# songrise/AvatarCraft

Measured on AMD Instinct MI355X. Metric: rays/sec, 4096-ray batch, 256x256 render (64+64 samples/ray), higher is better.
Workload: dtype f32

## Files before the change

avatarcraft_amd/csrc/nsr_device.hpp:

```cpp
#pragma once
#include "ac_common.hpp"
#include "ac_devmath.hpp"
#include "ac_sp_table.hpp"
#include "ac_sh16.hpp"
#include <type_traits>

using namespace acdev;

typedef float f32x4 __attribute__((ext_vector_type(4)));

namespace {

#ifndef AC_WPB
#define AC_WPB 8
#endif
constexpr int WAVES_PER_BLOCK = AC_WPB;
constexpr int BLOCK = WAVES_PER_BLOCK * 64;
#ifndef AC_MAXT
#define AC_MAXT 128
#endif
constexpr int MAXT = AC_MAXT;
constexpr int SEG_STATE = MAXT + 16 + 64;
#ifndef AC_ENC_ROUND
#define AC_ENC_ROUND 2
#endif

constexpr int OFF_W1F = 0;
constexpr int OFF_W2F = OFF_W1F + 4 * 9 * 64;
constexpr int OFF_C1F = OFF_W2F + 16 * 64;
constexpr int OFF_C2F = OFF_C1F + 4 * 6 * 64;
constexpr int OFF_C3F = OFF_C2F + 4 * 16 * 64;
constexpr int OFF_B1 = OFF_C3F + 16 * 64;
constexpr int OFF_B2 = OFF_B1 + 64;
constexpr int OFF_LVL = OFF_B2 + 16;
constexpr int OFF_LIN = OFF_LVL + 16 * 8;
constexpr int SPQ_FLOATS = 129 * 4;
constexpr int OFF_SPQ = OFF_LIN + 80;
constexpr int OFF_WAVE = OFF_SPQ + SPQ_FLOATS;
constexpr int FE_SLAB = 6 * 8 * 64;
constexpr int OFF_W1H = OFF_WAVE;
constexpr int OFF_W1L = OFF_W1H + 4 * 64 * 4;
constexpr int OFF_W1C = OFF_W1L + 4 * 64 * 4;
constexpr int CF_FRAGS = 14, CF_FRAG = 64 * 4;
constexpr int OFF_CFH = OFF_C1F;
constexpr int OFF_CFL = OFF_C1F + CF_FRAGS * CF_FRAG;
constexpr int OFF_C3L = OFF_W1C + 3 * 64;
static_assert(OFF_CFL + 12 * CF_FRAG == OFF_B1, "the bf16 colour fragments fill the fp32 colour region exactly");
constexpr int OFF_RWAVE = OFF_C3L + 2 * CF_FRAG;
constexpr int CF_OVERLAY = OFF_B1 - OFF_C1F;
constexpr int UPS_FLOATS = MAXT + 2 * MAXT + MAXT + 32;
constexpr int SLAB_ACC = MAXT + (FE_SLAB > UPS_FLOATS ? FE_SLAB : UPS_FLOATS);
constexpr int SLAB_SHB = SLAB_ACC + 16;
constexpr int WAVE_SLAB = SLAB_SHB + 80;
constexpr int LDS_FLOATS = OFF_RWAVE + WAVES_PER_BLOCK * WAVE_SLAB;
static_assert(LDS_FLOATS * 4 <= 160 * 1024, "LDS budget: one workgroup per CU");
static_assert(OFF_WAVE % 4 == 0 && OFF_RWAVE % 4 == 0 && WAVE_SLAB % 4 == 0, "16-byte aligned slabs");

#ifdef AC_PROFILE
#define AC_T0() unsigned long long t_prof_ = __builtin_amdgcn_s_memtime(); const unsigned long long ray_r0_ = __builtin_amdgcn_s_memrealtime()
#define AC_TICK(SLOT) { const unsigned long long t2_ = __builtin_amdgcn_s_memtime(); prof_acc[SLOT] += t2_ - t_prof_; t_prof_ = t2_; }
#else
#define AC_T0()
#define AC_TICK(SLOT)
#endif

struct LevelRec { float scale; uint32_t my, mz, offset, mask, hashed, wsize, pad; };

struct RenderArgs {
    const float *table;
    uint32_t table_bytes;
    const float *W1, *b1, *W2, *b2, *Wc1, *Wc2, *Wc3;
    const float *Wsh;
    const float *prepared;
    const float *rays_o, *rays_d, *bg, *noise, *lin_z, *lin_u;
    ac_render_out out;
    LevelRec lvl[16];
    int n_rays, T0, nup;
    int jmode[4];
    int jfine[4];
    float bound, two_bound, inv_s, car, one_m_car, eps;
    float inv_tb;
    const float *inv_s_dev;
    int fast;
    int skip_masked;
    int opacity_only;
    int perturb;
    unsigned long long *prof;
    const float *near_m, *far_m;
    const float *ext_pts;
    const uint8_t *mask;
    uint32_t *ray_counter;
    uint32_t *seg_flags;
    float *seg_state;
    uint64_t seg_cb;
    int seg_n;
    int pair_n;
    uint32_t *done_counter;
    uint32_t *handoff_timeouts;
    float *eik_red;
    uint32_t gen;
    int ex_from;
    int ex_rows;
    const uint8_t *ray_dead;
    float *zbuf;
    float *mid_pts;
};

enum { MODE_FULL = 0, MODE_UPSAMPLE = 2, MODE_FINAL = 3 };

__device__ __forceinline__ void cube_near_far(float ox, float oy, float oz, float dx, float dy, float dz, float bound, float &near, float &far)
{
    const float ex = dx + 1e-15f, ey = dy + 1e-15f, ez = dz + 1e-15f;
    const float ax = (-bound - ox) / ex, bx = (bound - ox) / ex;
    const float ay = (-bound - oy) / ey, by = (bound - oy) / ey;
    const float az = (-bound - oz) / ez, bz = (bound - oz) / ez;
    const float lx = ax < bx ? ax : bx, hx = ax > bx ? ax : bx;
    const float ly = ay < by ? ay : by, hy = ay > by ? ay : by;
    const float lz = az < bz ? az : bz, hz = az > bz ? az : bz;
    near = lx; if (ly > near) near = ly; if (lz > near) near = lz;
    far = hx; if (hy < far) far = hy; if (hz < far) far = hz;
    if (near < 0.05f) near = 0.05f;
}
__device__ __forceinline__ bool is_inf(float v) { return __builtin_fabsf(v) == __builtin_inff(); }

__device__ __forceinline__ void wave_sync()
{
    __builtin_amdgcn_fence(__ATOMIC_ACQ_REL, "wavefront");
    __builtin_amdgcn_wave_barrier();
}

template <int OFF> __device__ __forceinline__ float dpp_shr(float ident, float v)
{
    return __builtin_bit_cast(float, __builtin_amdgcn_update_dpp(__builtin_bit_cast(int, ident), __builtin_bit_cast(int, v),
                                                                  0x110 + OFF, 0xf, 0xf, false));
}
template <bool MUL> __device__ __forceinline__ float row_scan(float v)
{
    const float id = MUL ? 1.0f : 0.0f;
    float s;
    s = dpp_shr<1>(id, v); v = MUL ? s * v : s + v;
    s = dpp_shr<2>(id, v); v = MUL ? s * v : s + v;
    s = dpp_shr<4>(id, v); v = MUL ? s * v : s + v;
    s = dpp_shr<8>(id, v); v = MUL ? s * v : s + v;
    return v;
}
__device__ __forceinline__ float lane_bcast(float v, int lane)
{
    return __builtin_bit_cast(float, __builtin_amdgcn_readlane(__builtin_bit_cast(int, v), lane));
// ... 758 lines not shown
```

avatarcraft_amd/csrc/render_fused.hip:

```cpp
#include <atomic>
#include <map>
#include <mutex>
#include "nsr_device.hpp"

namespace {

#ifndef AC_XCD_CHUNK
#define AC_XCD_CHUNK 512
#endif
#define AC_RENDER_KERNEL render_rays_kernel
#define AC_RENDER_H16 false
#include "render_rays_kernel.hpp"
#undef AC_RENDER_KERNEL
#undef AC_RENDER_H16
#define AC_RENDER_KERNEL render_rays_h16_kernel
#define AC_RENDER_H16 true
#include "render_rays_kernel.hpp"
#undef AC_RENDER_KERNEL
#undef AC_RENDER_H16

__global__ __launch_bounds__(BLOCK) void field_sdf_kernel(const RenderArgs a, const float *__restrict__ x, uint32_t B,
                                                          float *__restrict__ out16)
{
    extern __shared__ __attribute__((aligned(16))) float lds[];
    fill_lds(lds, a);
    __syncthreads();
    const int lane = threadIdx.x & 63, wave = threadIdx.x >> 6, n = lane & 15, g = lane >> 4;
    const FieldCtx fc = make_ctx(a);
    const uint32_t ntiles = (B + 15) / 16;
    for (uint32_t tile = blockIdx.x * WAVES_PER_BLOCK + wave; tile < ntiles; tile += gridDim.x * WAVES_PER_BLOCK) {
        const uint32_t b = tile * 16 + n, bb = b < B ? b : B - 1;
        const float px = x[3 * bb], py = x[3 * bb + 1], pz = x[3 * bb + 2];
        const f32x4 o = sdf_tile(lds, fc, lane, px, py, pz);
        if (b < B) *reinterpret_cast<f32x4 *>(out16 + (size_t)b * 16 + 4 * g) = o;
    }
}

__global__ __launch_bounds__(BLOCK) void field_color_kernel(const RenderArgs a, const float *__restrict__ x, const float *__restrict__ dirs,
                                                            const float *__restrict__ nrm, const float *__restrict__ sdfout,
                                                            uint32_t B, float *__restrict__ rgb_out)
{
    extern __shared__ __attribute__((aligned(16))) float lds[];
    fill_lds(lds, a);
    __syncthreads();
    const int lane = threadIdx.x & 63, wave = threadIdx.x >> 6, n = lane & 15, g = lane >> 4;
    const uint32_t ntiles = (B + 15) / 16;
    float *slab = lds + OFF_WAVE + wave * 1024;
    for (uint32_t tile = blockIdx.x * WAVES_PER_BLOCK + wave; tile < ntiles; tile += gridDim.x * WAVES_PER_BLOCK) {
        const uint32_t b = tile * 16 + n, bb = b < B ? b : B - 1;
        const f32x4 so = *reinterpret_cast<const f32x4 *>(sdfout + (size_t)bb * 16 + 4 * g);
        float rgb[3];
        if (dirs) {
            wave_sync();
            sample_sh_bias(slab, a.Wsh, dirs[3 * bb], dirs[3 * bb + 1], dirs[3 * bb + 2], lane);
            color_tile(lds, lane, x[3 * bb], x[3 * bb + 1], x[3 * bb + 2], nrm[3 * bb], nrm[3 * bb + 1], nrm[3 * bb + 2], so, rgb, slab + 4 * lane, 256);
        } else
        color_tile(lds, lane, x[3 * bb], x[3 * bb + 1], x[3 * bb + 2], nrm[3 * bb], nrm[3 * bb + 1], nrm[3 * bb + 2], so, rgb);
        if (b < B && g == 0) { rgb_out[3 * b] = rgb[0]; rgb_out[3 * b + 1] = rgb[1]; rgb_out[3 * b + 2] = rgb[2]; }
    }
}

__global__ __launch_bounds__(BLOCK) void field_prepare_kernel(const RenderArgs a, float *__restrict__ image)
// ... 42 lines not shown
    const int ray = idx / T0, i = idx - ray * T0;
    const float ox = rays_o[3 * ray], oy = rays_o[3 * ray + 1], oz = rays_o[3 * ray + 2];
    const float dx = rays_d[3 * ray], dy = rays_d[3 * ray + 1], dz = rays_d[3 * ray + 2];
    float near, far;
    cube_near_far(ox, oy, oz, dx, dy, dz, bound, near, far);
    if (near_m) {
        const float nm = near_m[ray], fm = far_m[ray];
        if (!is_inf(nm)) near = nm;
        if (!is_inf(fm)) far = fm;
    }
    const float span = far - near;
    const float sample_dist = span / (float)T0;
    float zi = near + span * lin_z[i];
    if (perturb) zi = zi + (noise[idx] - 0.5f) * sample_dist;
    pts[3 * (size_t)idx] = ox + dx * zi; pts[3 * (size_t)idx + 1] = oy + dy * zi; pts[3 * (size_t)idx + 2] = oz + dz * zi;
}

static int check_render_args(const char *who, const ac_render_opts *op, const float *rays_o, const float *rays_d, const float *noise,
                             const float *lin_z, const float *lin_u, const ac_render_out *out)
{
    if (op->num_steps % 16 || op->upsample_steps % 16 || op->num_steps < 16 || op->num_steps > 64 ||
        op->upsample_steps < 0 || op->num_steps + op->upsample_steps > MAXT) {
        ac::set_error("%s: num_steps=%d upsample_steps=%d unsupported (multiples of 16, num_steps<=64, sum<=128)", who,
                      op->num_steps, op->upsample_steps);
        return AC_ERR_BAD_ARG;
    }
    if (!(op->fd_eps > 0.0f)) {
        ac::set_error("%s: fd_eps = %g (normal_epsilon_ratio >= 1): the finite-difference normals divide by it, it must be positive", who, (double)op->fd_eps);
        return AC_ERR_BAD_ARG;
    }
    if (op->n_rays <= 0) return AC_OK;
    if (!rays_o || !rays_d || !lin_z || (op->upsample_steps && !lin_u) || (op->perturb && !noise) || !out->image ||
        !out->weights_sum || !out->depth || !out->normal_map || !out->eik) {
        ac::set_error("%s: NULL buffer", who); return AC_ERR_BAD_ARG;
    }
    return AC_OK;
}

static int fill_render_args(RenderArgs &a, const ac_field *field, const ac_render_opts *op, const float *rays_o, const float *rays_d,
                            const float *bg, const float *noise, const float *lin_z, const float *lin_u, const ac_render_out *out)
{
    if (int rc = fill_render_common(a, field, op, rays_o, rays_d, bg, noise, lin_z, lin_u)) return rc;
    a.out = *out;
    a.pair_n = 0; a.ex_from = 0; a.ex_rows = op->n_rays;
    if (op->precision != 0 && op->precision != 1) { ac::set_error("ac_render_opts: precision %d unknown (0 = exact, 1 = fast)", op->precision); return AC_ERR_BAD_ARG; }
    if (op->skip_masked != 0 && op->skip_masked != 1) { ac::set_error("ac_render_opts: skip_masked must be 0 or 1"); return AC_ERR_BAD_ARG; }
    a.skip_masked = op->skip_masked;
    if (op->opacity_only != 0 && op->opacity_only != 1) { ac::set_error("ac_render_opts: opacity_only must be 0 or 1"); return AC_ERR_BAD_ARG; }
    a.opacity_only = op->opacity_only;
    if ((op->near_m != nullptr) != (op->far_m != nullptr)) { ac::set_error("ac_render_opts: near_m and far_m go together"); return AC_ERR_BAD_ARG; }
    return AC_OK;
}

#ifndef AC_RAY_SEGMENTS
#define AC_RAY_SEGMENTS 4
#endif
struct SegSlot { char *p; size_t bytes; uint32_t gen; uint64_t last_use; };
constexpr size_t SEG_POOL_MAX = 32;
static std::mutex g_seg_mu;
static std::map<std::pair<int, hipStream_t>, SegSlot> g_seg_pool;
static uint64_t g_seg_clock = 0;
static char *seg_scratch(size_t need, uint32_t &gen, hipStream_t stream)
{
    std::mutex &mu = g_seg_mu;
    auto &pool = g_seg_pool;
    int dev = 0;
    if (hipGetDevice(&dev) != hipSuccess || dev < 0) dev = 0;
    std::lock_guard<std::mutex> lock(mu);
    const auto key = std::make_pair(dev, stream);
    if (pool.find(key) == pool.end() && pool.size() >= SEG_POOL_MAX) {
        auto victim = pool.begin();
        for (auto it = pool.begin(); it != pool.end(); ++it) if (it->second.last_use < victim->second.last_use) victim = it;
        if (victim->second.p) (void)hipFree(victim->second.p);
        pool.erase(victim);
    }
    SegSlot &sl = pool[key];
    sl.last_use = ++g_seg_clock;
    if (sl.bytes < need) {
        if (sl.p) (void)hipFree(sl.p);
        sl.p = nullptr; sl.bytes = 0; sl.gen = 0;
        const size_t want = (need + ((size_t)1 << 20) - 1) & ~(((size_t)1 << 20) - 1);
        if (hipMalloc(reinterpret_cast<void **>(&sl.p), want) != hipSuccess) { sl.p = nullptr; return nullptr; }
        if (hipMemsetAsync(sl.p, 0, want, stream) != hipSuccess) { (void)hipFree(sl.p); sl.p = nullptr; return nullptr; }
        sl.bytes = want;
    }
    sl.gen = (sl.gen + 1u) & 0x0fffffffu;
    if (sl.gen == 0u) {
        if (hipMemsetAsync(sl.p, 0, sl.bytes, stream) != hipSuccess) return nullptr;
        sl.gen = 1u;
    }
    gen = sl.gen;
    return sl.p;
}

AC_API int ac_render_handoff_timeouts(ac_stream_t stream, uint32_t *count)
{
    if (!count) { ac::set_error("render_handoff_timeouts: NULL count"); return AC_ERR_BAD_ARG; }
    *count = 0;
    int dev = 0;
    if (hipGetDevice(&dev) != hipSuccess || dev < 0) dev = 0;
    char *p = nullptr;
    {
        std::lock_guard<std::mutex> lock(g_seg_mu);
        auto it = g_seg_pool.find(std::make_pair(dev, (hipStream_t)stream));
        if (it != g_seg_pool.end()) p = it->second.p;
    }
    if (!p) return AC_OK;
    if (hipMemcpyAsync(count, p + 260, sizeof(uint32_t), hipMemcpyDeviceToHost, (hipStream_t)stream) != hipSuccess ||
        hipStreamSynchronize((hipStream_t)stream) != hipSuccess) { ac::set_error("render_handoff_timeouts: copy failed"); return AC_ERR_LAUNCH; }
    return AC_OK;
}

template <int MODE, bool FAST, bool EX, bool SH = false, bool H16 = false>
static void launch_render_p(const RenderArgs &a, hipStream_t stream)
{
    const auto kernel = H16 ? render_rays_h16_kernel<MODE, FAST, EX, SH> : render_rays_kernel<MODE, FAST, EX, SH>;
    int blocks = (a.n_rays + WAVES_PER_BLOCK - 1) / WAVES_PER_BLOCK;
    static uint64_t seen = 0;
    const size_t lds_bytes = LDS_FLOATS * sizeof(float);
    ac::allow_dynamic_lds(seen, reinterpret_cast<const void *>(kernel), lds_bytes);
    RenderArgs b = a;
    {
        const int nt = (a.T0 + 16 * a.nup) / 16;
        int sn = (MODE != MODE_FULL) ? 1 : (nt < AC_RAY_SEGMENTS ? nt : AC_RAY_SEGMENTS);
        if (sn < 1) sn = 1;
        b.seg_n = sn; b.seg_cb = 0;
        for (int q = 0; q <= sn; ++q) b.seg_cb |= (uint64_t)((nt * q) / sn) << (4 * q);
        const size_t N = (size_t)a.n_rays, head = 512, flags = (N * 4 + 255) & ~(size_t)255;
        const size_t need = head + (sn > 1 ? flags + N * SEG_STATE * sizeof(float) : 0);
        uint32_t gen = 0;
        char *sc = seg_scratch(need, gen, stream);
        b.ray_counter = reinterpret_cast<uint32_t *>(sc);
        b.done_counter = sc ? reinterpret_cast<uint32_t *>(sc + 256) : nullptr;
        b.handoff_timeouts = sc ? reinterpret_cast<uint32_t *>(sc + 260) : nullptr;
        b.gen = gen;
        b.eik_red = (MODE == MODE_UPSAMPLE) ? nullptr : a.out.eik_reduced;
        b.seg_flags = sn > 1 ? reinterpret_cast<uint32_t *>(sc + head) : nullptr;
        b.seg_state = sn > 1 ? reinterpret_cast<float *>(sc + head + flags) : nullptr;
        const int cus = (int)ac::cu_count();
        if (blocks > cus) blocks = cus;
        blocks = (blocks + 7) & ~7;
        if (!sc) blocks = 0;
    }
    hipLaunchKernelGGL(kernel, dim3(blocks), dim3(BLOCK), lds_bytes, stream, b);
}
static bool wants_samples(const ac_render_out &o)
{
    return o.z_vals || o.weights || o.alpha || o.color || o.sdf || o.gradient || o.ss_inds || o.sort_index || o.sdf_out16 || o.pts || o.feat7;
}
template <int MODE>
static void launch_render(const RenderArgs &a, hipStream_t stream, bool h16 = false)
{
    const bool ex = wants_samples(a.out);
    if constexpr (MODE != MODE_UPSAMPLE) {
        dispatch_variants(a.fast, ex, a.Wsh != nullptr, [&](auto fast, auto ex_, auto sh) {
            if (h16) launch_render_p<MODE, decltype(fast)::value, decltype(ex_)::value, decltype(sh)::value, true>(a, stream);
            else launch_render_p<MODE, decltype(fast)::value, decltype(ex_)::value, decltype(sh)::value>(a, stream);
        });
        return;
    }
    const bool inds = a.out.ss_inds || a.out.sort_index;
    if (h16) { if (inds) launch_render_p<MODE, false, true, false, true>(a, stream); else launch_render_p<MODE, false, false, false, true>(a, stream); }
    else if (inds) launch_render_p<MODE, false, true>(a, stream);
    else launch_render_p<MODE, false, false>(a, stream);
}

__global__ __launch_bounds__(256) void table_to_half_kernel(const float2 *__restrict__ table, uint32_t n_entries, uint32_t *__restrict__ out, uint32_t *__restrict__ n_bad)
{
    uint32_t bad = 0;
    for (uint32_t i = blockIdx.x * blockDim.x + threadIdx.x; i < n_entries; i += gridDim.x * blockDim.x) {
        const float2 v = table[i];
        const _Float16 h0 = (_Float16)v.x, h1 = (_Float16)v.y;
        const uint32_t b0 = __builtin_bit_cast(unsigned short, h0), b1 = __builtin_bit_cast(unsigned short, h1);
        out[i] = b0 | (b1 << 16);
        const bool o0 = (b0 & 0x7fffu) == 0x7c00u && !is_inf(v.x), o1 = (b1 & 0x7fffu) == 0x7c00u && !is_inf(v.y);
        bad += (o0 || o1) ? 1u : 0u;
    }
    if (bad) atomicAdd(n_bad, bad);
}

AC_API int ac_table_to_half(const float *table, uint32_t n_entries, void *table_h16, uint32_t *n_bad, ac_stream_t stream)
{
    if (n_entries == 0) return AC_OK;
    if (!table || !table_h16 || !n_bad) { ac::set_error("table_to_half: NULL buffer"); return AC_ERR_BAD_ARG; }
    uint32_t blocks = (n_entries + 255u) / 256u;
    if (blocks > 4096u) blocks = 4096u;
    hipLaunchKernelGGL(table_to_half_kernel, dim3(blocks), dim3(256), 0, (hipStream_t)stream, reinterpret_cast<const float2 *>(table), n_entries,
                       static_cast<uint32_t *>(table_h16), n_bad);
    return ac::check_launch("table_to_half");
}

static int check_h16_args(const char *who, const ac_field *field, const void *table_h16, const ac_render_opts *op, const ac_render_out *out)
{
    if (!field) { ac::set_error("%s: NULL field", who); return AC_ERR_BAD_ARG; }
// ... 282 lines not shown
```

avatarcraft_amd/csrc/render_rays_kernel.hpp:

```cpp
template <int MODE, bool FAST, bool EX, bool SH = false>
__global__ __launch_bounds__(BLOCK) void AC_RENDER_KERNEL(const RenderArgs a)
{
    constexpr bool FC = FAST;
    extern __shared__ __attribute__((aligned(16))) float lds[];
    if (a.prepared) {
        const float4 *src = reinterpret_cast<const float4 *>(a.prepared);
        float4 *dst = reinterpret_cast<float4 *>(lds);
        for (int e = threadIdx.x; e < OFF_RWAVE / 4; e += blockDim.x)
            dst[e] = src[(FC && 4 * e >= OFF_C1F && 4 * e < OFF_B1) ? e + (OFF_RWAVE - OFF_C1F) / 4 : e];
        __syncthreads();
        for (int e = threadIdx.x; e < 64; e += blockDim.x) lds[OFF_LIN + e] = e < a.T0 ? a.lin_z[e] : 0.0f;
        for (int e = threadIdx.x; e < 16; e += blockDim.x) lds[OFF_LIN + 64 + e] = a.lin_u ? a.lin_u[e] : 0.0f;
    } else {
        fill_lds_sdf(lds, a);
        if constexpr (FAST) fill_lds_fast(lds, a);
        if constexpr (FC) fill_lds_color_fast<true, true>(lds, a);
        else fill_lds_color(lds, a);
    }
    __syncthreads();

    const int lane = threadIdx.x & 63, wave = threadIdx.x >> 6;
    const int n = lane & 15, g = lane >> 4;
    float *zs0 = lds + OFF_RWAVE + wave * WAVE_SLAB;
    float *zs1 = zs0 + MAXT;
    float *sd = zs1 + MAXT;
    float *cdf = sd + 2 * MAXT;
    float *znl = cdf + MAXT;
    float *fsl = zs1;
    const FieldCtx fc = make_ctx(a);
    const W2Row0 w2r0 = load_w2_row0(lds, lane);
    const float bound = a.bound;
    const float inv_s_core = a.inv_s_dev ? *a.inv_s_dev : a.inv_s;
    const int T0 = a.T0, nup = a.nup, T = T0 + 16 * nup;

#ifdef AC_PROFILE
    unsigned long long prof_acc[8] = {0, 0, 0, 0, 0, 0, 0, 0};
    const unsigned long long prof_t0 = __builtin_amdgcn_s_memtime(), prof_r0 = __builtin_amdgcn_s_memrealtime();
#endif
    int bid = blockIdx.x;
    {
        const int k = blockIdx.x & 7, q = gridDim.x >> 3, r = gridDim.x & 7;
        bid = k * q + (k < r ? k : r) + (blockIdx.x >> 3);
    }
#ifndef AC_START_STAGGER
#define AC_START_STAGGER 1
#endif
    if (a.n_rays >= 2048)
        for (int k_ = 0; k_ < AC_START_STAGGER * wave; ++k_) __builtin_amdgcn_s_sleep(64);
    const int xper = ((a.n_rays + 7) / 8 + 7) & ~7, xchunk = xper < AC_XCD_CHUNK ? xper : AC_XCD_CHUNK, xcd = blockIdx.x & 7;
    const int seg_n = (MODE == MODE_UPSAMPLE) ? 1 : a.seg_n;
    for (int seg = 0; seg < seg_n; ++seg) {
    const int c_begin = (MODE == MODE_UPSAMPLE) ? 0 : (int)((a.seg_cb >> (4 * seg)) & 15u), c_end = (MODE == MODE_UPSAMPLE) ? 0 : (int)((a.seg_cb >> (4 * seg + 4)) & 15u);
    const bool seg_first = seg == 0, seg_last = seg + 1 == seg_n;
    for (;;) {
        int ray = 0;
        if (lane == 0) ray = (int)atomicAdd(a.ray_counter + xcd * 8 + seg, 1u);
        ray = __builtin_amdgcn_readfirstlane(ray);
        {
            const int k = ray / xchunk, base = (k * 8 + xcd) * xchunk;
            if (base >= a.n_rays) break;
            ray = base + (ray - k * xchunk);
            if (ray >= a.n_rays) continue;
        }
        int rin = ray;
        if (a.pair_n) { rin = ray >> 1; ray = rin + ((ray & 1) ? a.pair_n : 0); }
        (void)bid;
        const int exr = ray - a.ex_from;
        const bool ex_on = exr >= 0;
        AC_T0();
        const float ox = a.rays_o[3 * rin], oy = a.rays_o[3 * rin + 1], oz = a.rays_o[3 * rin + 2];
        const float dx = a.rays_d[3 * rin], dy = a.rays_d[3 * rin + 1], dz = a.rays_d[3 * rin + 2];
        float near, far;
        cube_near_far(ox, oy, oz, dx, dy, dz, bound, near, far);
        if (a.near_m) {
            const float nm = a.near_m[rin], fm = a.far_m[rin];
            if (!is_inf(nm)) near = nm;
            if (!is_inf(fm)) far = fm;
        }
        const float span = far - near;
        const float sample_dist = span / (float)T0;
        int cur = (MODE == MODE_FINAL) ? 0 : (nup & 1), cnt = T0;
        float *const zs_first = cur ? zs1 : zs0;

        if constexpr (MODE == MODE_UPSAMPLE) {
            if (a.ray_dead && a.ray_dead[ray]) {
                for (int i = lane; i < T; i += 64) {
                    const int ic = i < T0 ? i : T0 - 1;
                    float zi = near + span * lds[OFF_LIN + ic];
                    if (a.perturb) zi = zi + (a.noise[(size_t)ray * T0 + ic] - 0.5f) * sample_dist;
                    const size_t si = (size_t)ray * T + i;
                    a.zbuf[si] = zi;
                    if (a.mid_pts) { a.mid_pts[3 * si] = ox + dx * zi; a.mid_pts[3 * si + 1] = oy + dy * zi; a.mid_pts[3 * si + 2] = oz + dz * zi; }
                }
                wave_sync();
                continue;
            }
        }
        if constexpr (MODE == MODE_FINAL) {
            for (int i = lane; i < T; i += 64) zs0[i] = a.zbuf[(size_t)ray * T + i];
        } else if (seg_first) {
            for (int c = 0; c < T0 / 16; ++c) {
                const int i = 16 * c + n;
                float zi = near + span * lds[OFF_LIN + i];
                if (a.perturb) zi = zi + (a.noise[(size_t)ray * T0 + i] - 0.5f) * sample_dist;
                if (nup > 0) {
                    float px, py, pz;
                    if (MODE == MODE_UPSAMPLE && a.ext_pts) {
                        const float *e = a.ext_pts + ((size_t)ray * T0 + i) * 3;
                        px = clampf(e[0], -bound, bound); py = clampf(e[1], -bound, bound); pz = clampf(e[2], -bound, bound);
                    } else {
                        px = clampf(ox + dx * zi, -bound, bound); py = clampf(oy + dy * zi, -bound, bound);
                        pz = clampf(oz + dz * zi, -bound, bound);
                    }
                    const f32x4 o2 = sdf_tile<AC_RENDER_H16>(lds, fc, lane, px, py, pz);
                    if (g == 0) sd[cur * MAXT + i] = o2[0];
                }
                if (g == 0) zs_first[i] = zi;
            }
        }
        wave_sync();
        AC_TICK(0)
// ... 97 lines not shown
#pragma unroll
            for (int ch = 0; ch < 2; ++ch) {
                const int i = 64 * ch + lane;
                if (i < cnt) {
                    const float zi = zc[i];
                    int c = 0;
#pragma unroll
                    for (int j = 0; j < 16; ++j) c += (znl[j] < zi) ? 1 : 0;
                    int before = i;
                    if (!old_sorted) {
                        before = 0;
                        for (int k = 0; k < cnt; ++k) { const float zk = zc[k]; before += ((zk < zi) || (zk == zi && k < i)) ? 1 : 0; }
                    }
                    zn_[before + c] = zi; sn_[before + c] = sc[i];
                    if (sidx) sidx[before + c] = i;
                }
                if (sidx && i >= cnt + 16) sidx[i] = -1;
            }
            if (g == 0) {
                int lo = 0, hi = cnt;
                if (old_sorted) {
                    while (lo < hi) { const int md = (lo + hi) >> 1; if (zc[md] <= znew) lo = md + 1; else hi = md; }
                } else {
                    for (int k = 0; k < cnt; ++k) lo += (zc[k] <= znew) ? 1 : 0;
                }
                int c = 0;
#pragma unroll
                for (int j = 0; j < 16; ++j) { const float zj = znl[j]; c += ((zj < znew) || (zj == znew && j < n)) ? 1 : 0; }
                zn_[lo + c] = znew; sn_[lo + c] = sdf_new;
                if (sidx) sidx[lo + c] = cnt + n;
            }
            cnt += 16; cur ^= 1;
            wave_sync();
            AC_TICK(1)
        }

        const float *zf = zs0;
        if constexpr (MODE == MODE_UPSAMPLE) {
            for (int i = lane; i < T; i += 64) {
                const float zi = zf[i];
                const float delta = (i < T - 1) ? zf[i + 1] - zi : sample_dist;
                const float zmid = (i < T - 1) ? zi + 0.5f * delta : zi;
                const size_t si = (size_t)ray * T + i;
                a.zbuf[si] = zi;
                if (a.mid_pts) { a.mid_pts[3 * si] = ox + dx * zmid; a.mid_pts[3 * si + 1] = oy + dy * zmid; a.mid_pts[3 * si + 2] = oz + dz * zmid; }
            }
            wave_sync();
            continue;
        }
        float cT = 1.0f;
        float *const accs = zs0 + SLAB_ACC;
        if constexpr (SH && MODE != MODE_UPSAMPLE) { if (seg_first && !a.opacity_only) ray_sh_bias(zs0 + SLAB_SHB, a.Wsh, dx, dy, dz, lane); }
        if (!seg_first) {
            int timed_out = 0;
            if (lane == 0) {
                int spins = 0;
                for (;;) {
                    const uint32_t f = __hip_atomic_load(a.seg_flags + ray, __ATOMIC_RELAXED, __HIP_MEMORY_SCOPE_AGENT);
                    if (((f >> 4) == a.gen && (f & 15u) >= (uint32_t)seg) || spins >= (1 << 21)) break;
                    __builtin_amdgcn_s_sleep(8); ++spins;
                }
                timed_out = spins >= (1 << 21);
                if (timed_out && a.handoff_timeouts) atomicAdd(a.handoff_timeouts, 1u);
            }
            timed_out = __builtin_amdgcn_readfirstlane(timed_out);
            wave_sync();
            const uint32_t *st = reinterpret_cast<const uint32_t *>(a.seg_state + (size_t)ray * SEG_STATE);
            if constexpr (MODE != MODE_FINAL)
                for (int i = lane; i < T; i += 64) zs0[i] = __uint_as_float(__hip_atomic_load(st + i, __ATOMIC_RELAXED, __HIP_MEMORY_SCOPE_AGENT));
            const float cv = __uint_as_float(__hip_atomic_load(st + MAXT + (lane & 15), __ATOMIC_RELAXED, __HIP_MEMORY_SCOPE_AGENT));
            cT = lane_bcast(cv, 0);
            if (lane < 16) accs[lane] = cv;
            if constexpr (SH) zs0[SLAB_SHB + lane] = __uint_as_float(__hip_atomic_load(st + MAXT + 16 + lane, __ATOMIC_RELAXED, __HIP_MEMORY_SCOPE_AGENT));
            if (timed_out) {
                cT = __builtin_nanf("");
                if (lane < 16) accs[lane] = cT;
            }
            wave_sync();
        }
        const float bxe = a.eps;
        const int c_hi = c_end < T / 16 ? c_end : T / 16;
        for (int c = c_begin; c < c_hi; ++c) {
            const int i = 16 * c + n;
            const float zi = zf[i];
            const float delta = (i < T - 1) ? zf[i + 1] - zi : sample_dist;
            const float zmid = (i < T - 1) ? zi + 0.5f * delta : zi;
            float px, py, pz;
            if constexpr (MODE == MODE_FINAL) {
                const float *e = a.ext_pts + ((size_t)ray * T + i) * 3;
                px = clampf(e[0], -bound, bound); py = clampf(e[1], -bound, bound); pz = clampf(e[2], -bound, bound);
            } else {
                px = clampf(ox + dx * zmid, -bound, bound); py = clampf(oy + dy * zmid, -bound, bound);
                pz = clampf(oz + dz * zmid, -bound, bound);
            }
            AC_TICK(7)
            bool skip = false;
            if constexpr (MODE == MODE_FINAL) {
                if (a.skip_masked) skip = __ballot(a.mask[(size_t)ray * T + i] != 0) == 0ull;
            }
            f32x4 oc = { 0.0f, 0.0f, 0.0f, 0.0f };
            float gr[3] = { 0.0f, 0.0f, 0.0f };
            if (!skip) {
            float fe0[4][2];
            encode_stencil<AC_RENDER_H16>(lds, fsl, fc, lane, px, py, pz, bxe, fe0);
            if (EX && ex_on && a.out.feat7) {
                int lane_x = lane;
                asm volatile("" : "+v"(lane_x));
                f32x4 *dst = reinterpret_cast<f32x4 *>(a.out.feat7) + (((size_t)exr * (T / 16) + (i >> 4)) * 14) * 64 + lane_x;
                dst[0] = f32x4{ fe0[0][0], fe0[0][1], fe0[1][0], fe0[1][1] };
                dst[64] = f32x4{ fe0[2][0], fe0[2][1], fe0[3][0], fe0[3][1] };
#pragma unroll 1
                for (int e = 0; e < 6; ++e) {
                    const float *sp = fsl + (e * 8) * 64 + lane;
                    dst[(2 * e + 2) * 64] = f32x4{ sp[0], sp[64], sp[128], sp[192] };
                    dst[(2 * e + 3) * 64] = f32x4{ sp[256], sp[320], sp[384], sp[448] };
                }
            }
            AC_TICK(3)
            const float pc0 = sel4(g, px, py, pz, 0.0f);
            float spos = 0.0f;
            if constexpr (FAST) {
                const Acc4 acc0 = sdf_l1(lds, lane, pc0, fe0);
                oc = sdf_l2(lds, lane, acc0);
#pragma unroll 1
                for (int e = 0; e < 6; ++e) {
                    const int kn = e >> 1;
                    float fe[4][2];
#pragma unroll
                    for (int q_ = 0; q_ < 8; ++q_) fe[q_ >> 1][q_ & 1] = fsl[(e * 8 + q_) * 64 + lane];
                    const float pk = kn == 0 ? px : (kn == 1 ? py : pz);
                    const float poff = clampf(pk + ((e & 1) ? -bxe : bxe), -bound, bound);
                    const Acc4 acc = sdf_l1_delta(lds, lane, acc0, fe, fe0, kn, poff - pk);
                    const float s_e = sdf_l2_sdf(lds, acc, w2r0);
                    if (!(e & 1)) spos = s_e;
                    else {
                        const float gk = 0.5f * (spos - s_e) / bxe;
                        if (kn == 0) gr[0] = gk; else if (kn == 1) gr[1] = gk; else gr[2] = gk;
                    }
                }
            } else {
            Acc4 acc = sdf_l1(lds, lane, pc0, fe0);
#pragma unroll 1
            for (int e = 0; e < 7; ++e) {
                Acc4 accn = acc;
                if (e < 6) {
                    const int kn = e >> 1;
                    float fe[4][2];
#pragma unroll
                    for (int q_ = 0; q_ < 8; ++q_) fe[q_ >> 1][q_ & 1] = fsl[(e * 8 + q_) * 64 + lane];
                    const float pk = kn == 0 ? px : (kn == 1 ? py : pz);
                    const float poff = clampf(pk + ((e & 1) ? -bxe : bxe), -bound, bound);
                    accn = sdf_l1(lds, lane, g == kn ? poff : pc0, fe);
                }
                if (e == 0) oc = sdf_l2(lds, lane, acc);
                else {
                    const float s_e = sdf_l2_sdf(lds, acc, w2r0);
                    const int k = (e - 1) >> 1;
                    if (e & 1) spos = s_e;
                    else {
                        const float gk = 0.5f * (spos - s_e) / bxe;
                        if (k == 0) gr[0] = gk; else if (k == 1) gr[1] = gk; else gr[2] = gk;
                    }
                }
                acc = accn;
            }
            }
            }
            AC_TICK(4)
            const float gx = gr[0], gy = gr[1], gz = gr[2];
            const FdNormal nrm = fd_normal(gx, gy, gz);
            const float gn = nrm.gn, nx = nrm.nx, ny = nrm.ny, nz = nrm.nz;
            float rgb[3] = { 0.0f, 0.0f, 0.0f };
            if (!skip && !a.opacity_only) {
                if constexpr (FC) color_tile_fast(lds, lane, px, py, pz, nx, ny, nz, oc, rgb, nullptr, 16, SH ? zs0 + SLAB_SHB : nullptr);
                else color_tile(lds, lane, px, py, pz, nx, ny, nz, oc, rgb, nullptr, 16, SH ? zs0 + SLAB_SHB : nullptr);
            }
            AC_TICK(5)
            const float sdf0 = oc[0];
            float alpha = neus_alpha(lds, a, (dx * nx + dy * ny) + dz * nz, sdf0, delta, inv_s_core);
            if constexpr (MODE == MODE_FINAL) alpha = alpha * (a.mask[(size_t)ray * T + i] ? 1.0f : 0.0f);
            const float om = 1.0f - alpha + 1e-7f;
            const float loc = row_scan<true>(om);
            const float sh = dpp_shr<1>(1.0f, loc);
            float Tex;
            if (n == 0) Tex = (c == 0) ? 1.0f : cT;
            else Tex = (c == 0) ? sh : cT * sh;
            const float tot = lane_bcast(loc, 15);
            cT = (c == 0) ? tot : cT * tot;
            const float wgt = alpha * Tex;
            const float zn01 = clampf((zi - near) / span, 0.0f, 1.0f);
            const float pn = __builtin_sqrtf((px * px + py * py) + pz * pz);
            const float relax = (pn < 1.2f && !skip) ? 1.0f : 0.0f;
            const float eerr = relax * ((gn - 1.0f) * (gn - 1.0f));
            {
                const float t1 = row_scan<false>(wgt), t2 = row_scan<false>(rgb[0] * wgt), t3 = row_scan<false>(rgb[1] * wgt), t4 = row_scan<false>(rgb[2] * wgt),
                            t5 = row_scan<false>(nx * wgt), t6 = row_scan<false>(ny * wgt), t7 = row_scan<false>(nz * wgt), t8 = row_scan<false>(wgt * zn01),
                            t9 = row_scan<false>(eerr), t10 = row_scan<false>(relax);
                if (lane == 15) {
#define AC_ACC(K, T_) accs[K] = (c == 0) ? T_ : accs[K] + T_;
                    AC_ACC(1, t1) AC_ACC(2, t2) AC_ACC(3, t3) AC_ACC(4, t4) AC_ACC(5, t5) AC_ACC(6, t6) AC_ACC(7, t7) AC_ACC(8, t8) AC_ACC(9, t9) AC_ACC(10, t10)
#undef AC_ACC
                }
            }
            AC_TICK(6)
            if (g == 0) {
                const size_t si = (size_t)exr * T + i;
                if (EX && ex_on && a.out.z_vals) a.out.z_vals[si] = zi;
                if (EX && ex_on && a.out.weights) a.out.weights[si] = wgt;
                if (EX && ex_on && a.out.alpha) a.out.alpha[si] = alpha;
                if (EX && ex_on && a.out.sdf) a.out.sdf[si] = sdf0;
                if (EX && ex_on && a.out.color) { a.out.color[3 * si] = rgb[0]; a.out.color[3 * si + 1] = rgb[1]; a.out.color[3 * si + 2] = rgb[2]; }
                if (EX && ex_on && a.out.gradient) { a.out.gradient[3 * si] = gx; a.out.gradient[3 * si + 1] = gy; a.out.gradient[3 * si + 2] = gz; }
                if (EX && ex_on && a.out.pts) { a.out.pts[3 * si] = px; a.out.pts[3 * si + 1] = py; a.out.pts[3 * si + 2] = pz; }
            }
            if (EX && ex_on && a.out.sdf_out16) {
                int g_x = g;
                asm volatile("" : "+v"(g_x));
                *reinterpret_cast<f32x4 *>(a.out.sdf_out16 + ((size_t)exr * T + i) * 16 + 4 * g_x) = oc;
            }
        }
        if (!seg_last) {
            uint32_t *st = reinterpret_cast<uint32_t *>(a.seg_state + (size_t)ray * SEG_STATE);
            if (MODE != MODE_FINAL && seg_first)
                for (int i = lane; i < T; i += 64) __hip_atomic_store(st + i, __float_as_uint(zf[i]), __ATOMIC_RELAXED, __HIP_MEMORY_SCOPE_AGENT);
            wave_sync();
            if (lane < 11) {
                const float cv = lane == 0 ? cT : accs[lane];
                __hip_atomic_store(st + MAXT + lane, __float_as_uint(cv), __ATOMIC_RELAXED, __HIP_MEMORY_SCOPE_AGENT);
            }
            if constexpr (SH) { if (seg_first) __hip_atomic_store(st + MAXT + 16 + lane, __float_as_uint(zs0[SLAB_SHB + lane]), __ATOMIC_RELAXED, __HIP_MEMORY_SCOPE_AGENT); }
            asm volatile("s_waitcnt vmcnt(0)" ::: "memory");
            wave_sync();
            if (lane == 0) __hip_atomic_store(a.seg_flags + ray, (a.gen << 4) | (uint32_t)(seg + 1), __ATOMIC_RELAXED, __HIP_MEMORY_SCOPE_AGENT);
            wave_sync();
            continue;
        }
        wave_sync();
        if (lane == 0) {
            const float s_w = accs[1], s_r = accs[2], s_g = accs[3], s_b = accs[4], s_nx = accs[5], s_ny = accs[6], s_nz = accs[7], s_d = accs[8], s_en = accs[9], s_ed = accs[10];
            const float b0 = a.bg ? a.bg[3 * ray] : 1.0f, b1 = a.bg ? a.bg[3 * ray + 1] : 1.0f, b2 = a.bg ? a.bg[3 * ray + 2] : 1.0f;
            a.out.image[3 * ray] = s_r + (1.0f - s_w) * b0;
            a.out.image[3 * ray + 1] = s_g + (1.0f - s_w) * b1;
            a.out.image[3 * ray + 2] = s_b + (1.0f - s_w) * b2;
            a.out.normal_map[3 * ray] = s_nx; a.out.normal_map[3 * ray + 1] = s_ny; a.out.normal_map[3 * ray + 2] = s_nz;
            a.out.weights_sum[ray] = s_w;
            a.out.depth[ray] = s_d;
            a.out.eik[2 * ray] = s_en; a.out.eik[2 * ray + 1] = s_ed;
        }
        wave_sync();
#ifdef AC_PROFILE
        if (a.prof && lane == 0) a.prof[(size_t)a.n_rays * 10 + ray] = __builtin_amdgcn_s_memrealtime() - ray_r0_;
#endif
    }
    }
    const __attribute__((address_space(4))) RenderArgs *ka = (const __attribute__((address_space(4))) RenderArgs *)__builtin_amdgcn_kernarg_segment_ptr();
    asm volatile("" : "+s"(ka));
    uint32_t *const k_done = ka->done_counter;
    if (k_done) {
        __syncthreads();
        uint32_t *ldsu = reinterpret_cast<uint32_t *>(lds);
        if (threadIdx.x == 0) {
            __threadfence();
            ldsu[0] = atomicAdd(k_done, 1u) == gridDim.x - 1u ? 1u : 0u;
        }
        __syncthreads();
        const bool last = ldsu[0] != 0u;
        __syncthreads();
        if (last) {
            __threadfence();
            float *const k_red = ka->eik_red;
            const int k_pair = ka->pair_n, k_n = ka->n_rays;
            const float *const k_eik = ka->out.eik;
            uint32_t *const k_cnt = ka->ray_counter;
            if (k_red) {
                const int nred = k_pair ? 2 : 1, nper = k_pair ? k_pair : k_n;
                float *pn = lds, *pd = lds + 1024;
                for (int q = 0; q < nred; ++q) {
                    const float *e = k_eik + (size_t)q * nper * 2;
                    for (int t = (int)threadIdx.x; t < 1024; t += BLOCK) {
                        float sa = 0.0f, sb = 0.0f;
                        for (int r = t; r < nper; r += 1024) { sa += e[2 * r]; sb += e[2 * r + 1]; }
                        pn[t] = sa; pd[t] = sb;
                    }
                    __syncthreads();
                    for (int st = 512; st > 0; st >>= 1) {
                        for (int t = (int)threadIdx.x; t < st; t += BLOCK) { pn[t] += pn[t + st]; pd[t] += pd[t + st]; }
                        __syncthreads();
                    }
                    if (threadIdx.x == 0) { k_red[2 * q] = pn[0] / (pd[0] + 1e-5f); k_red[2 * q + 1] = pd[0] + 1e-5f; }
                    __syncthreads();
                }
            }
            if (threadIdx.x < 64) k_cnt[threadIdx.x] = 0u;
            if (threadIdx.x == 64) *k_done = 0u;
        }
    }
#ifdef AC_PROFILE
    if (a.prof && lane == 0) { const int w_ = blockIdx.x * WAVES_PER_BLOCK + wave; for (int i = 0; i < 8; ++i) a.prof[w_ * 10 + i] = prof_acc[i];
        a.prof[w_ * 10 + 8] = __builtin_amdgcn_s_memtime() - prof_t0; a.prof[w_ * 10 + 9] = __builtin_amdgcn_s_memrealtime() - prof_r0; }
#endif
}
```

Measured before the change: 5.436 million.

## Schedule ray segments from a precomputed per-XCD work list with ticket prefetch

Replaces the fixed uniform 4-way segment split, with one atomic counter per segment, by a host-built work list per XCD. The list orders items segment-major using an uneven tile split (3/2/2/1 by default), and each wave takes items through a single ticket counter. The next ticket is fetched during the last tile of the current item, which hides the atomic and item-load latency. The aim is better load balance and less handoff waiting between the segments of a ray. In exchange it adds host-side list building, caching and upload, and the wait/handoff ordering now depends on the list order.

Measured after the change: 5.507 million, median of 6. 1.01x the previous value.

```diff
diff --git a/avatarcraft_amd/csrc/nsr_device.hpp b/avatarcraft_amd/csrc/nsr_device.hpp
--- a/avatarcraft_amd/csrc/nsr_device.hpp
+++ b/avatarcraft_amd/csrc/nsr_device.hpp
@@ -59,9 +59,13 @@
 #ifdef AC_PROFILE
 #define AC_T0() unsigned long long t_prof_ = __builtin_amdgcn_s_memtime(); const unsigned long long ray_r0_ = __builtin_amdgcn_s_memrealtime()
 #define AC_TICK(SLOT) { const unsigned long long t2_ = __builtin_amdgcn_s_memtime(); prof_acc[SLOT] += t2_ - t_prof_; t_prof_ = t2_; }
+#define AC_BND_MARK() prof_bm = __builtin_amdgcn_s_memtime()
+#define AC_BND_TICK(SLOT) { const unsigned long long t3_ = __builtin_amdgcn_s_memtime(); prof_bnd[SLOT] += t3_ - prof_bm; prof_bm = t3_; }
 #else
 #define AC_T0()
 #define AC_TICK(SLOT)
+#define AC_BND_MARK()
+#define AC_BND_TICK(SLOT)
 #endif
 
 struct LevelRec { float scale; uint32_t my, mz, offset, mask, hashed, wsize, pad; };
@@ -92,8 +96,7 @@
     uint32_t *ray_counter;
     uint32_t *seg_flags;
     float *seg_state;
-    uint64_t seg_cb;
-    int seg_n;
+    const uint32_t *work_list;
     int pair_n;
     uint32_t *done_counter;
     uint32_t *handoff_timeouts;
diff --git a/avatarcraft_amd/csrc/render_fused.hip b/avatarcraft_amd/csrc/render_fused.hip
--- a/avatarcraft_amd/csrc/render_fused.hip
+++ b/avatarcraft_amd/csrc/render_fused.hip
@@ -1,13 +1,13 @@
+#include <algorithm>
 #include <atomic>
 #include <map>
 #include <mutex>
+#include <vector>
 #include "nsr_device.hpp"
+#include "render_worklist.hpp"
 
 namespace {
 
-#ifndef AC_XCD_CHUNK
-#define AC_XCD_CHUNK 512
-#endif
 #define AC_RENDER_KERNEL render_rays_kernel
 #define AC_RENDER_H16 false
 #include "render_rays_kernel.hpp"
@@ -156,14 +156,50 @@
     return AC_OK;
 }
 
-#ifndef AC_RAY_SEGMENTS
-#define AC_RAY_SEGMENTS 4
-#endif
-struct SegSlot { char *p; size_t bytes; uint32_t gen; uint64_t last_use; };
+struct WorkList { int n_rays, tiles, pair_n, waves; uint32_t *dev, *host; hipEvent_t uploaded; uint64_t last_use; };
+constexpr size_t WORKLISTS_PER_SLOT = 4;
+struct SegSlot { char *p; size_t bytes; uint32_t gen; uint64_t last_use; std::vector<WorkList> lists; };
 constexpr size_t SEG_POOL_MAX = 32;
 static std::mutex g_seg_mu;
 static std::map<std::pair<int, hipStream_t>, SegSlot> g_seg_pool;
 static uint64_t g_seg_clock = 0;
+static void free_worklist(WorkList &w)
+{
+    if (w.uploaded) { (void)hipEventSynchronize(w.uploaded); (void)hipEventDestroy(w.uploaded); }
+    if (w.dev) (void)hipFree(w.dev);
+    if (w.host) (void)hipHostFree(w.host);
+    w.dev = w.host = nullptr; w.uploaded = nullptr;
+}
+static const uint32_t *seg_worklist(int n_rays, int tiles, int pair_n, int waves, hipStream_t stream)
+{
+    int dev = 0;
+    if (hipGetDevice(&dev) != hipSuccess || dev < 0) dev = 0;
+    std::lock_guard<std::mutex> lock(g_seg_mu);
+    auto it = g_seg_pool.find(std::make_pair(dev, stream));
+    if (it == g_seg_pool.end()) return nullptr;
+    std::vector<WorkList> &ls = it->second.lists;
+    for (WorkList &w : ls)
+        if (w.n_rays == n_rays && w.tiles == tiles && w.pair_n == pair_n && w.waves == waves) { w.last_use = ++g_seg_clock; return w.dev; }
+    if (ls.size() >= WORKLISTS_PER_SLOT) {
+        size_t v = 0;
+        for (size_t i = 1; i < ls.size(); ++i) if (ls[i].last_use < ls[v].last_use) v = i;
+        free_worklist(ls[v]);
+        ls.erase(ls.begin() + (long)v);
+    }
+    std::vector<uint32_t> words;
+    ac_worklist::build(n_rays, tiles, pair_n, waves, AC_WORKLIST_POLICY, words);
+    WorkList w{ n_rays, tiles, pair_n, waves, nullptr, nullptr, nullptr, ++g_seg_clock };
+    const size_t bytes = words.size() * sizeof(uint32_t);
+    if (hipMalloc(reinterpret_cast<void **>(&w.dev), bytes) != hipSuccess) { w.dev = nullptr; (void)hipGetLastError(); return nullptr; }
+    if (hipHostMalloc(reinterpret_cast<void **>(&w.host), bytes, hipHostMallocDefault) != hipSuccess) { w.host = nullptr; (void)hipGetLastError(); free_worklist(w); return nullptr; }
+    std::copy(words.begin(), words.end(), w.host);
+    if (hipEventCreateWithFlags(&w.uploaded, hipEventDisableTiming) != hipSuccess) { w.uploaded = nullptr; free_worklist(w); return nullptr; }
+    if (hipMemcpyAsync(w.dev, w.host, bytes, hipMemcpyHostToDevice, stream) != hipSuccess || hipEventRecord(w.uploaded, stream) != hipSuccess) {
+        (void)hipStreamSynchronize(stream); free_worklist(w); return nullptr;
+    }
+    ls.push_back(w);
+    return w.dev;
+}
 static char *seg_scratch(size_t need, uint32_t &gen, hipStream_t stream)
 {
     std::mutex &mu = g_seg_mu;
@@ -176,6 +212,7 @@
         auto victim = pool.begin();
         for (auto it = pool.begin(); it != pool.end(); ++it) if (it->second.last_use < victim->second.last_use) victim = it;
         if (victim->second.p) (void)hipFree(victim->second.p);
+        for (WorkList &w : victim->second.lists) free_worklist(w);
         pool.erase(victim);
     }
     SegSlot &sl = pool[key];
@@ -226,24 +263,23 @@
     RenderArgs b = a;
     {
         const int nt = (a.T0 + 16 * a.nup) / 16;
-        int sn = (MODE != MODE_FULL) ? 1 : (nt < AC_RAY_SEGMENTS ? nt : AC_RAY_SEGMENTS);
-        if (sn < 1) sn = 1;
-        b.seg_n = sn; b.seg_cb = 0;
-        for (int q = 0; q <= sn; ++q) b.seg_cb |= (uint64_t)((nt * q) / sn) << (4 * q);
+        const bool listed = MODE == MODE_FULL;
         const size_t N = (size_t)a.n_rays, head = 512, flags = (N * 4 + 255) & ~(size_t)255;
-        const size_t need = head + (sn > 1 ? flags + N * SEG_STATE * sizeof(float) : 0);
+        const size_t need = head + (listed ? flags + N * SEG_STATE * sizeof(float) : 0);
         uint32_t gen = 0;
         char *sc = seg_scratch(need, gen, stream);
+        const int cus = (int)ac::cu_count();
+        if (blocks > cus) blocks = cus;
+        blocks = (blocks + 7) & ~7;
+        b.work_list = (listed && sc) ? seg_worklist(a.n_rays, nt, a.pair_n, (blocks / 8) * WAVES_PER_BLOCK, stream) : nullptr;
+        if (listed && !b.work_list) sc = nullptr;
         b.ray_counter = reinterpret_cast<uint32_t *>(sc);
         b.done_counter = sc ? reinterpret_cast<uint32_t *>(sc + 256) : nullptr;
         b.handoff_timeouts = sc ? reinterpret_cast<uint32_t *>(sc + 260) : nullptr;
         b.gen = gen;
         b.eik_red = (MODE == MODE_UPSAMPLE) ? nullptr : a.out.eik_reduced;
-        b.seg_flags = sn > 1 ? reinterpret_cast<uint32_t *>(sc + head) : nullptr;
-        b.seg_state = sn > 1 ? reinterpret_cast<float *>(sc + head + flags) : nullptr;
-        const int cus = (int)ac::cu_count();
-        if (blocks > cus) blocks = cus;
-        blocks = (blocks + 7) & ~7;
+        b.seg_flags = (listed && sc) ? reinterpret_cast<uint32_t *>(sc + head) : nullptr;
+        b.seg_state = (listed && sc) ? reinterpret_cast<float *>(sc + head + flags) : nullptr;
         if (!sc) blocks = 0;
     }
     hipLaunchKernelGGL(kernel, dim3(blocks), dim3(BLOCK), lds_bytes, stream, b);
diff --git a/avatarcraft_amd/csrc/render_rays_kernel.hpp b/avatarcraft_amd/csrc/render_rays_kernel.hpp
--- a/avatarcraft_amd/csrc/render_rays_kernel.hpp
+++ b/avatarcraft_amd/csrc/render_rays_kernel.hpp
@@ -36,6 +36,7 @@
 #ifdef AC_PROFILE
     unsigned long long prof_acc[8] = {0, 0, 0, 0, 0, 0, 0, 0};
     const unsigned long long prof_t0 = __builtin_amdgcn_s_memtime(), prof_r0 = __builtin_amdgcn_s_memrealtime();
+    unsigned long long prof_bnd[2] = {0, 0}, prof_bm = prof_t0;
 #endif
     int bid = blockIdx.x;
     {
@@ -47,26 +48,38 @@
 #endif
     if (a.n_rays >= 2048)
         for (int k_ = 0; k_ < AC_START_STAGGER * wave; ++k_) __builtin_amdgcn_s_sleep(64);
-    const int xper = ((a.n_rays + 7) / 8 + 7) & ~7, xchunk = xper < AC_XCD_CHUNK ? xper : AC_XCD_CHUNK, xcd = blockIdx.x & 7;
-    const int seg_n = (MODE == MODE_UPSAMPLE) ? 1 : a.seg_n;
-    for (int seg = 0; seg < seg_n; ++seg) {
-    const int c_begin = (MODE == MODE_UPSAMPLE) ? 0 : (int)((a.seg_cb >> (4 * seg)) & 15u), c_end = (MODE == MODE_UPSAMPLE) ? 0 : (int)((a.seg_cb >> (4 * seg + 4)) & 15u);
-    const bool seg_first = seg == 0, seg_last = seg + 1 == seg_n;
+    constexpr bool LISTED = MODE == MODE_FULL;
+    const int xchunk = ac_worklist::xcd_chunk(a.n_rays), xcd = blockIdx.x & 7;
+    uint32_t *const tk_counter = a.ray_counter + xcd * 8;
+    const __attribute__((address_space(4))) uint32_t *const wl = (const __attribute__((address_space(4))) uint32_t *)a.work_list;
+    uint32_t wl_cnt = 0;
+    const __attribute__((address_space(4))) uint32_t *wl_items = wl;
+    if constexpr (LISTED) { wl_cnt = wl[ac_worklist::XCDS + xcd]; wl_items = wl + ac_worklist::HEADER_WORDS + 2 * (size_t)wl[xcd]; }
+#define AC_TAKE_TICKET(TK) { uint32_t v_ = 0; if (lane == 0) v_ = atomicAdd(tk_counter, 1u); TK = (uint32_t)__builtin_amdgcn_readfirstlane((int)v_); }
+#define AC_FETCH_ITEM(TK, W0, W1) { W0 = 0u; W1 = 0u; if (TK < wl_cnt) { W0 = wl_items[2 * (size_t)TK]; W1 = wl_items[2 * (size_t)TK + 1]; } }
+    uint32_t tk = 0, it_ray = 0, it_meta = 0;
+    if constexpr (LISTED) { AC_TAKE_TICKET(tk) AC_FETCH_ITEM(tk, it_ray, it_meta) }
     for (;;) {
-        int ray = 0;
-        if (lane == 0) ray = (int)atomicAdd(a.ray_counter + xcd * 8 + seg, 1u);
-        ray = __builtin_amdgcn_readfirstlane(ray);
-        {
-            const int k = ray / xchunk, base = (k * 8 + xcd) * xchunk;
-            if (base >= a.n_rays) break;
-            ray = base + (ray - k * xchunk);
-            if (ray >= a.n_rays) continue;
+        int ray = 0, c_begin = 0, c_end = MAXT / 16, seq = 0;
+        bool seg_first = true, seg_last = true;
+        bool tk_ahead = false;
+        if constexpr (LISTED) {
+            if (tk >= wl_cnt) break;
+            ray = (int)it_ray;
+            c_begin = ac_worklist::meta_begin(it_meta); c_end = ac_worklist::meta_end(it_meta); seq = ac_worklist::meta_seq(it_meta);
+            seg_first = (it_meta & ac_worklist::META_SAMPLING) != 0u; seg_last = (it_meta & ac_worklist::META_LAST) != 0u;
+        } else {
+            AC_TAKE_TICKET(tk)
+            ray = ac_worklist::ticket_to_work(a.n_rays, xchunk, xcd, (int)tk);
+            if (ray == ac_worklist::TICKET_END) break;
+            if (ray == ac_worklist::TICKET_GAP) continue;
         }
         int rin = ray;
-        if (a.pair_n) { rin = ray >> 1; ray = rin + ((ray & 1) ? a.pair_n : 0); }
+        if (LISTED && a.pair_n && ray >= a.pair_n) rin = ray - a.pair_n;
         (void)bid;
         const int exr = ray - a.ex_from;
         const bool ex_on = exr >= 0;
+        AC_BND_TICK(0)
         AC_T0();
         const float ox = a.rays_o[3 * rin], oy = a.rays_o[3 * rin + 1], oz = a.rays_o[3 * rin + 2];
         const float dx = a.rays_d[3 * rin], dy = a.rays_d[3 * rin + 1], dz = a.rays_d[3 * rin + 2];
@@ -270,12 +283,13 @@
         float *const accs = zs0 + SLAB_ACC;
         if constexpr (SH && MODE != MODE_UPSAMPLE) { if (seg_first && !a.opacity_only) ray_sh_bias(zs0 + SLAB_SHB, a.Wsh, dx, dy, dz, lane); }
         if (!seg_first) {
+            AC_BND_MARK();
             int timed_out = 0;
             if (lane == 0) {
                 int spins = 0;
                 for (;;) {
                     const uint32_t f = __hip_atomic_load(a.seg_flags + ray, __ATOMIC_RELAXED, __HIP_MEMORY_SCOPE_AGENT);
-                    if (((f >> 4) == a.gen && (f & 15u) >= (uint32_t)seg) || spins >= (1 << 21)) break;
+                    if (((f >> 4) == a.gen && (f & 15u) >= (uint32_t)seq) || spins >= (1 << 21)) break;
                     __builtin_amdgcn_s_sleep(8); ++spins;
                 }
                 timed_out = spins >= (1 << 21);
@@ -295,6 +309,7 @@
                 if (lane < 16) accs[lane] = cT;
             }
             wave_sync();
+            AC_BND_TICK(1)
         }
         const float bxe = a.eps;
         const int c_hi = c_end < T / 16 ? c_end : T / 16;
@@ -318,6 +333,7 @@
             }
             f32x4 oc = { 0.0f, 0.0f, 0.0f, 0.0f };
             float gr[3] = { 0.0f, 0.0f, 0.0f };
+            uint32_t tk_v = 0;
             if (!skip) {
             float fe0[4][2];
             encode_stencil<AC_RENDER_H16>(lds, fsl, fc, lane, px, py, pz, bxe, fe0);
@@ -385,6 +401,13 @@
             }
             }
             AC_TICK(4)
+            if constexpr (LISTED) {
+                if (c + 1 == c_hi && lane == 0) {
+                    __attribute__((address_space(1))) uint32_t *tk_p = (__attribute__((address_space(1))) uint32_t *)tk_counter;
+                    asm volatile("" : "+v"(tk_p));
+                    tk_v = __hip_atomic_fetch_add(tk_p, 1u, __ATOMIC_RELAXED, __HIP_MEMORY_SCOPE_AGENT);
+                }
+            }
             const float gx = gr[0], gy = gr[1], gz = gr[2];
             const FdNormal nrm = fd_normal(gx, gy, gz);
             const float gn = nrm.gn, nx = nrm.nx, ny = nrm.ny, nz = nrm.nz;
@@ -421,6 +444,9 @@
                 }
             }
             AC_TICK(6)
+            if constexpr (LISTED) {
+                if (c + 1 == c_hi) { tk = (uint32_t)__builtin_amdgcn_readfirstlane((int)tk_v); AC_FETCH_ITEM(tk, it_ray, it_meta) tk_ahead = true; }
+            }
             if (g == 0) {
                 const size_t si = (size_t)exr * T + i;
                 if (EX && ex_on && a.out.z_vals) a.out.z_vals[si] = zi;
@@ -437,6 +463,7 @@
                 *reinterpret_cast<f32x4 *>(a.out.sdf_out16 + ((size_t)exr * T + i) * 16 + 4 * g_x) = oc;
             }
         }
+        AC_BND_MARK();
         if (!seg_last) {
             uint32_t *st = reinterpret_cast<uint32_t *>(a.seg_state + (size_t)ray * SEG_STATE);
             if (MODE != MODE_FINAL && seg_first)
@@ -449,8 +476,9 @@
             if constexpr (SH) { if (seg_first) __hip_atomic_store(st + MAXT + 16 + lane, __float_as_uint(zs0[SLAB_SHB + lane]), __ATOMIC_RELAXED, __HIP_MEMORY_SCOPE_AGENT); }
             asm volatile("s_waitcnt vmcnt(0)" ::: "memory");
             wave_sync();
-            if (lane == 0) __hip_atomic_store(a.seg_flags + ray, (a.gen << 4) | (uint32_t)(seg + 1), __ATOMIC_RELAXED, __HIP_MEMORY_SCOPE_AGENT);
-            wave_sync();
+            if (lane == 0) __hip_atomic_store(a.seg_flags + ray, (a.gen << 4) | (uint32_t)(seq + 1), __ATOMIC_RELAXED, __HIP_MEMORY_SCOPE_AGENT);
+            wave_sync();
+            if constexpr (LISTED) { if (!tk_ahead) { AC_TAKE_TICKET(tk) AC_FETCH_ITEM(tk, it_ray, it_meta) } }
             continue;
         }
         wave_sync();
@@ -469,8 +497,10 @@
 #ifdef AC_PROFILE
         if (a.prof && lane == 0) a.prof[(size_t)a.n_rays * 10 + ray] = __builtin_amdgcn_s_memrealtime() - ray_r0_;
 #endif
+        if constexpr (LISTED) { if (!tk_ahead) { AC_TAKE_TICKET(tk) AC_FETCH_ITEM(tk, it_ray, it_meta) } }
     }
-    }
+#undef AC_TAKE_TICKET
+#undef AC_FETCH_ITEM
     const __attribute__((address_space(4))) RenderArgs *ka = (const __attribute__((address_space(4))) RenderArgs *)__builtin_amdgcn_kernarg_segment_ptr();
     asm volatile("" : "+s"(ka));
     uint32_t *const k_done = ka->done_counter;
@@ -515,6 +545,7 @@
     }
 #ifdef AC_PROFILE
     if (a.prof && lane == 0) { const int w_ = blockIdx.x * WAVES_PER_BLOCK + wave; for (int i = 0; i < 8; ++i) a.prof[w_ * 10 + i] = prof_acc[i];
+        a.prof[(size_t)a.n_rays * 11 + 2 * w_] = prof_bnd[0]; a.prof[(size_t)a.n_rays * 11 + 2 * w_ + 1] = prof_bnd[1];
         a.prof[w_ * 10 + 8] = __builtin_amdgcn_s_memtime() - prof_t0; a.prof[w_ * 10 + 9] = __builtin_amdgcn_s_memrealtime() - prof_r0; }
 #endif
 }
diff --git a/avatarcraft_amd/csrc/render_worklist.hpp b/avatarcraft_amd/csrc/render_worklist.hpp
--- /dev/null
+++ b/avatarcraft_amd/csrc/render_worklist.hpp
@@ -0,0 +1,107 @@
+#pragma once
+#include <cstdint>
+#include <vector>
+
+#if defined(__HIPCC__) || defined(__CUDACC__)
+#define AC_WL_HD __host__ __device__ inline
+#else
+#define AC_WL_HD inline
+#endif
+
+#ifndef AC_XCD_CHUNK
+#define AC_XCD_CHUNK 512
+#endif
+#ifndef AC_WORKLIST_POLICY
+#define AC_WORKLIST_POLICY 1
+#endif
+
+namespace ac_worklist {
+
+constexpr int XCDS = 8;
+constexpr int MAX_ITEMS = 8;
+constexpr int HEADER_WORDS = 16;
+
+constexpr uint32_t META_SAMPLING = 1u << 12, META_LAST = 1u << 13;
+struct Item { uint32_t ray, meta; };
+AC_WL_HD uint32_t make_meta(int c_begin, int c_end, int seq, bool sampling, bool last)
+{
+    return (uint32_t)c_begin | ((uint32_t)c_end << 4) | ((uint32_t)seq << 8) | (sampling ? META_SAMPLING : 0u) | (last ? META_LAST : 0u);
+}
+AC_WL_HD int meta_begin(uint32_t m) { return (int)(m & 15u); }
+AC_WL_HD int meta_end(uint32_t m) { return (int)((m >> 4) & 15u); }
+AC_WL_HD int meta_seq(uint32_t m) { return (int)((m >> 8) & 15u); }
+
+AC_WL_HD int xcd_chunk(int n_rays)
+{
+    const int xper = ((n_rays + 7) / 8 + 7) & ~7;
+    return xper < AC_XCD_CHUNK ? xper : AC_XCD_CHUNK;
+}
+enum { TICKET_END = -2, TICKET_GAP = -1 };
+AC_WL_HD int ticket_to_work(int n_rays, int xchunk, int xcd, int t)
+{
+    const int k = t / xchunk, base = (k * XCDS + xcd) * xchunk;
+    if (base >= n_rays) return TICKET_END;
+    const int w = base + (t - k * xchunk);
+    return w < n_rays ? w : TICKET_GAP;
+}
+AC_WL_HD int work_to_ray(int w, int pair_n) { return pair_n ? (w >> 1) + ((w & 1) ? pair_n : 0) : w; }
+
+constexpr int N_POLICIES = 9;
+inline const int *policy_split(int policy, bool first_round, int local)
+{
+    static const int s2222[] = { 2, 2, 2, 2, 0 }, s3221[] = { 3, 2, 2, 1, 0 }, s22211[] = { 2, 2, 2, 1, 1, 0 }, s13211[] = { 1, 3, 2, 1, 1, 0 }, s31211[] = { 3, 1, 2, 1, 1, 0 },
+                     s332[] = { 3, 3, 2, 0 }, s4211[] = { 4, 2, 1, 1, 0 }, s3311[] = { 3, 3, 1, 1, 0 }, s431[] = { 4, 3, 1, 0 };
+    switch (policy) {
+    case 1: return s3221;
+    case 2: return s22211;
+    case 3: return first_round ? s2222 : s22211;
+    case 4: return first_round ? s2222 : ((local & 1) ? s31211 : s13211);
+    case 5: return s332;
+    case 6: return s4211;
+    case 7: return s3311;
+    case 8: return s431;
+    default: return s2222;
+    }
+}
+inline int split_bounds(const int *split8, int tiles, int b[MAX_ITEMS + 1])
+{
+    int n = 0, cum = 0;
+    b[0] = 0;
+    for (int q = 0; split8[q]; ++q) {
+        cum += split8[q];
+        const int e = (tiles * cum) / 8;
+        if (e > b[n]) b[++n] = e;
+    }
+    return n;
+}
+
+inline void build(int n_rays, int tiles, int pair_n, int waves_per_xcd, int policy, std::vector<uint32_t> &out)
+{
+    out.assign(HEADER_WORDS, 0u);
+    if (n_rays <= 0 || tiles < 1) return;
+    if (tiles > 15) tiles = 15;
+    const int xchunk = xcd_chunk(n_rays);
+    std::vector<int> rays;
+    uint32_t n_items = 0;
+    for (int xcd = 0; xcd < XCDS; ++xcd) {
+        rays.clear();
+        for (int t = 0;; ++t) {
+            const int w = ticket_to_work(n_rays, xchunk, xcd, t);
+            if (w == TICKET_END) break;
+            if (w != TICKET_GAP) rays.push_back(w);
+        }
+        out[xcd] = n_items;
+        for (int seq = 0; seq < MAX_ITEMS; ++seq)
+            for (int local = 0; local < (int)rays.size(); ++local) {
+                int b[MAX_ITEMS + 1];
+                const int n = split_bounds(policy_split(policy, local < waves_per_xcd, local), tiles, b);
+                if (seq >= n) continue;
+                out.push_back((uint32_t)work_to_ray(rays[local], pair_n));
+                out.push_back(make_meta(b[seq], b[seq + 1], seq, seq == 0, seq + 1 == n));
+                ++n_items;
+            }
+        out[XCDS + xcd] = n_items - out[xcd];
+    }
+}
+
+}
```
